# hao-ai-lab/LookaheadDecoding

Measured on NVIDIA H100. Metric: tokens/sec (wall-clock) and accepted-tokens/step, Llama-2-7B W=15 N=5 G=15, higher is better.
Workload: dtype bf16

## Files before the change

lookaheaddecoding_b200/csrc/attn_tc.cu:

```cuda
#include "tc_common.cuh"

#include <cstdlib>
#include <mutex>
#include <type_traits>
#include <unordered_map>

namespace lade {

constexpr int TC_BM = 128;
constexpr int TC_BN = 128;
constexpr int TC_D = 128;
constexpr int TC_STAGES = 3;
constexpr int TC_CONSUMER_THREADS = 256;
constexpr int TC_THREADS = TC_CONSUMER_THREADS + 32;
constexpr int TC_TILE_BYTES = 128 * 128 * 2;
constexpr int TC_HALF_BYTES = TC_TILE_BYTES / 2;
constexpr int TC_SMEM_TILES = TC_TILE_BYTES * (1 + 2 * TC_STAGES);
constexpr int TC_SMEM_BYTES = TC_SMEM_TILES + 256 + 1024;
constexpr float TC_LOG2E = 1.4426950408889634f;
constexpr int TC_MAX_COUNTERS = 16384;

__device__ long long* g_attn_timing = nullptr;
__device__ __forceinline__ long long global_ns() {
  unsigned long long t;
  asm volatile("mov.u64 %0, %%globaltimer;" : "=l"(t));
  return (long long)t;
}
__device__ __forceinline__ int sm_id() {
  int s;
  asm volatile("mov.u32 %0, %%smid;" : "=r"(s));
  return s;
}
#define TC_STAMP(slot, tid) do { if (tbuf && threadIdx.x == (tid)) tbuf[slot] = global_ns(); } while (0)
enum { TS_START = 0, TS_KFULL0 = 1, TS_SFULL0 = 2, TS_OFINAL = 3, TS_STAGED = 4, TS_TICKET = 5, TS_END = 7, TS_SMID = 15 };

template <typename ET> __device__ __forceinline__ float2 unpack2(uint32_t u);
template <> __device__ __forceinline__ float2 unpack2<__nv_bfloat16>(uint32_t u) {
  return make_float2(__uint_as_float(u << 16), __uint_as_float(u & 0xffff0000u));
}
template <> __device__ __forceinline__ float2 unpack2<__half>(uint32_t u) {
  return __half22float2(*reinterpret_cast<__half2*>(&u));
}

template <typename ET>
__device__ __forceinline__ void qk_tile(float (&s)[64], uint32_t sQ_a, uint32_t sK_a, int wg) {
  wg_fence();
#pragma unroll
  for (int kb = 0; kb < 2; ++kb)
#pragma unroll
    for (int k = 0; k < 4; ++k) {
      const uint64_t da = wg_desc(sQ_a + kb * TC_HALF_BYTES + wg * 8192 + k * 32, 16, 1024);
      const uint64_t db = wg_desc(sK_a + kb * TC_HALF_BYTES + k * 32, 16, 1024);
      wgmma_m64n128_ss<ET>(s, da, db, (kb | k) ? 1u : 0u);
    }
  wg_commit();
  wg_wait_all();
  wg_fence_regs(s);
}

template <typename ET>
__device__ __forceinline__ void pv_tile(float (&o)[64], const uint32_t (&p)[32], uint32_t sV_a) {
  wg_fence_regs(o);
  wg_fence();
#pragma unroll
  for (int kk = 0; kk < 8; ++kk) wgmma_m64n128_rs_tb<ET>(o, p + 4 * kk, wg_desc(sV_a + kk * 2048, TC_HALF_BYTES, 1024));
  wg_commit();
  wg_wait_all();
  wg_fence_regs(o);
}

__device__ __forceinline__ void tile_mask(uint32_t (&mb)[2][4], const uint32_t* const (&mrow)[2], const int (&row)[2],
                                          int mask_words, int tile0, int kv_len, int q_len, int is_prefill) {
#pragma unroll
  for (int rr = 0; rr < 2; ++rr)
#pragma unroll
    for (int w = 0; w < 4; ++w)
      mb[rr][w] = (tile0 + 32 * w + 32 <= kv_len)
                      ? 0xffffffffu
                      : visible_bits32(mrow[rr], mask_words, tile0 + 32 * w, kv_len, q_len, is_prefill, row[rr]);
}
__device__ __forceinline__ bool vis(const uint32_t (&mb)[2][4], int rr, int i, int e, int t) {
  return (mb[rr][i >> 2] >> (8 * (i & 3) + 2 * t + e)) & 1u;
}

template <typename ET, bool REF>
__global__ void __launch_bounds__(TC_THREADS, 1)
attn_fwd_tc_kernel(const __grid_constant__ CUtensorMap tmQ, const __grid_constant__ CUtensorMap tmK,
                   const __grid_constant__ CUtensorMap tmV, ET* __restrict__ out,
                   const uint32_t* __restrict__ rowmask, int mask_words, const int* __restrict__ meta, int q_pad,
                   int n_heads, int n_kv_heads, int n_splits, float inv_sqrt_d, int* __restrict__ counters,
                   float2* __restrict__ part_ml, float* __restrict__ part_o) {
  extern __shared__ unsigned char smem_raw[];
  const uint32_t raw_a = smem_u32(smem_raw);
  const uint32_t sQ_a = (raw_a + 1023u) & ~1023u;
  unsigned char* smem = smem_raw + (sQ_a - raw_a);
  const int split = blockIdx.x, h = blockIdx.y, mt = blockIdx.z;
  const int warp = threadIdx.x >> 5, lane = threadIdx.x & 31;

  const int q_len = meta[LADE_M_Q_LEN];
  const int kv_len = meta[LADE_M_KV_LEN];
  const int is_prefill = meta[LADE_M_IS_PREFILL];
  const int T = kv_len + q_len;
  int Tm = T;
  if (is_prefill) Tm = min(T, kv_len + min(q_len, (mt + 1) * TC_BM));
  const int n_tiles = (Tm + TC_BN - 1) / TC_BN;
  const int t_base = n_tiles / n_splits, t_rem = n_tiles - t_base * n_splits;
  const int n_active = n_tiles < n_splits ? n_tiles : n_splits;
  const bool active = split < n_active;
  const int tile_lo = split * t_base + (split < t_rem ? split : t_rem);
  const int my_tiles = active ? t_base + (split < t_rem ? 1 : 0) : 0;
  if (REF && t_base + (t_rem ? 1 : 0) > TC_STAGES) __trap();
  const int hk = h / (n_heads / n_kv_heads);
  const int HD = n_heads * TC_D;
  const long long slab = (long long)n_heads * gridDim.z * TC_BM;
  const long long prow0 = ((long long)h * gridDim.z + mt) * TC_BM;
  const int n_wg = (mt * TC_BM + 64 < q_pad) ? 2 : 1;
  const bool zero_last = active && (tile_lo + my_tiles) * TC_BN > T;
  long long* tbuf = g_attn_timing ? g_attn_timing + 16ll * ((blockIdx.z * gridDim.y + blockIdx.y) * gridDim.x + blockIdx.x) : nullptr;
  TC_STAMP(TS_START, 0);
  if (tbuf && threadIdx.x == 0) tbuf[TS_SMID] = sm_id();
  griddep_launch_dependents();

  uint64_t* bars = reinterpret_cast<uint64_t*>(smem + TC_SMEM_TILES);
  const uint32_t bar0 = smem_u32(bars);
  auto BAR = [&](int i) { return bar0 + 8u * (uint32_t)i; };
  const int B_QFULL = 0, B_KFULL = 1, B_VFULL = 1 + TC_STAGES, B_FREE = 1 + 2 * TC_STAGES, B_VZERO = 1 + 3 * TC_STAGES;
  auto sK_a = [&](int s) { return sQ_a + (uint32_t)TC_TILE_BYTES * (1 + 2 * s); };
  auto sV_a = [&](int s) { return sQ_a + (uint32_t)TC_TILE_BYTES * (2 + 2 * s); };
  auto issue_tile = [&](int j) {
    const int s = j % TC_STAGES;
    const int row0 = (tile_lo + j) * TC_BN;
    mbar_expect_tx(BAR(B_KFULL + s), TC_TILE_BYTES);
    tma_load_3d(sK_a(s), &tmK, BAR(B_KFULL + s), 0, row0, hk);
    tma_load_3d(sK_a(s) + TC_HALF_BYTES, &tmK, BAR(B_KFULL + s), 64, row0, hk);
    mbar_expect_tx(BAR(B_VFULL + s), TC_TILE_BYTES);
    tma_load_3d(sV_a(s), &tmV, BAR(B_VFULL + s), 0, row0, hk);
    tma_load_3d(sV_a(s) + TC_HALF_BYTES, &tmV, BAR(B_VFULL + s), 64, row0, hk);
  };

  if (active && threadIdx.x == TC_CONSUMER_THREADS) {
    mbar_init(BAR(B_QFULL), 1);
    for (int s = 0; s < TC_STAGES; ++s) {
      mbar_init(BAR(B_KFULL + s), 1);
      mbar_init(BAR(B_VFULL + s), 1);
      mbar_init(BAR(B_FREE + s), 4 * n_wg);
    }
    mbar_init(BAR(B_VZERO), 1);
    fence_barrier_init();
    const int n_pre = my_tiles < TC_STAGES ? my_tiles : TC_STAGES;
    int n_old = 0;
    while (n_old < n_pre && (tile_lo + n_old + 1) * TC_BN <= kv_len) ++n_old;
    for (int j = 0; j < n_old; ++j) issue_tile(j);
    griddep_wait();
    mbar_expect_tx(BAR(B_QFULL), TC_TILE_BYTES);
    tma_load_3d(sQ_a, &tmQ, BAR(B_QFULL), 0, mt * TC_BM, h);
    tma_load_3d(sQ_a + TC_HALF_BYTES, &tmQ, BAR(B_QFULL), 64, mt * TC_BM, h);
    for (int j = n_old; j < n_pre; ++j) issue_tile(j);
  }
  __syncthreads();
  griddep_wait();

  const int wg = warp >> 2;
  const int g = lane >> 2, t = lane & 3;
  const int rl[2] = {wg * 64 + (warp & 3) * 16 + g, wg * 64 + (warp & 3) * 16 + g + 8};
  const bool work = active && warp < 8 && wg < n_wg;
  float o[64];
  float m_row[2] = {-INFINITY, -INFINITY}, l_row[2] = {0.f, 0.f};
#pragma unroll
  for (int i = 0; i < 64; ++i) o[i] = 0.f;

  if (warp == 8) {
    if (active) {
      if (lane == 0) {
        for (int j = TC_STAGES; j < my_tiles; ++j) {
          const int s = j % TC_STAGES;
          mbar_wait(BAR(B_FREE + s), ((j / TC_STAGES) - 1) & 1);
          issue_tile(j);
        }
      }
      __syncwarp();
      if (zero_last) {
        const int j = my_tiles - 1, s = j % TC_STAGES;
        const int r0 = T - (tile_lo + j) * TC_BN;
        mbar_wait(BAR(B_VFULL + s), (j / TC_STAGES) & 1);
        unsigned char* pV = smem + TC_TILE_BYTES * (2 + 2 * s);
        const uint4 z = make_uint4(0, 0, 0, 0);
        for (int c = r0 * 8 + lane; c < TC_BN * 8; c += 32) {
          const int r = c >> 3, cc = c & 7;
          *reinterpret_cast<uint4*>(pV + r * 128 + cc * 16) = z;
          *reinterpret_cast<uint4*>(pV + TC_HALF_BYTES + r * 128 + cc * 16) = z;
        }
        fence_proxy_async();
        __syncwarp();
        if (lane == 0) mbar_arrive(BAR(B_VZERO));
      }
    }
    if (REF) {
      cluster_arrive(); cluster_wait();
      cluster_arrive(); cluster_wait();
    }
  } else {
    const int row[2] = {mt * TC_BM + rl[0], mt * TC_BM + rl[1]};
    const uint32_t* const mrow[2] = {
        (row[0] < q_pad && !is_prefill && rowmask != nullptr) ? rowmask + (long long)row[0] * mask_words : nullptr,
        (row[1] < q_pad && !is_prefill && rowmask != nullptr) ? rowmask + (long long)row[1] * mask_words : nullptr};
    auto wait_v = [&](int j) {
      const int s = j % TC_STAGES;
      mbar_wait(BAR(B_VFULL + s), (j / TC_STAGES) & 1);
      if (zero_last && j == my_tiles - 1) mbar_wait(BAR(B_VZERO), 0);
    };
    if (work) mbar_wait(BAR(B_QFULL), 0);
    if (!REF) {
      for (int j = 0; work && j < my_tiles; ++j) {
        const int s = j % TC_STAGES;
        const int tile0 = (tile_lo + j) * TC_BN;
        mbar_wait(BAR(B_KFULL + s), (j / TC_STAGES) & 1);
        if (j == 0) TC_STAMP(TS_KFULL0, 0);
        float sc[64];
        qk_tile<ET>(sc, sQ_a, sK_a(s), wg);
        if (j == 0) TC_STAMP(TS_SFULL0, 0);
        uint32_t mb[2][4];
        tile_mask(mb, mrow, row, mask_words, tile0, kv_len, q_len, is_prefill);
        float off[2];
#pragma unroll
        for (int rr = 0; rr < 2; ++rr) {
          float mx = -INFINITY;
#pragma unroll
          for (int i = 0; i < 16; ++i)
#pragma unroll
            for (int e = 0; e < 2; ++e) mx = fmaxf(mx, vis(mb, rr, i, e, t) ? sc[4 * i + 2 * rr + e] : -INFINITY);
          mx = fmaxf(mx, __shfl_xor_sync(0xffffffffu, mx, 1));
          mx = fmaxf(mx, __shfl_xor_sync(0xffffffffu, mx, 2));
          const float mtile = mx == -INFINITY ? -INFINITY : round_to<ET>(round_to<ET>(mx) * inv_sqrt_d);
          if (mtile > m_row[rr]) {
            const float scale = m_row[rr] == -INFINITY ? 1.f : exp2f((m_row[rr] - mtile) * TC_LOG2E);
            l_row[rr] *= scale;
#pragma unroll
            for (int i = 0; i < 16; ++i) { o[4 * i + 2 * rr] *= scale; o[4 * i + 2 * rr + 1] *= scale; }
            m_row[rr] = mtile;
          }
          off[rr] = m_row[rr] == -INFINITY ? 0.f : m_row[rr] * TC_LOG2E;
        }
        uint32_t pa[32];
#pragma unroll
        for (int i = 0; i < 16; ++i)
#pragma unroll
          for (int rr = 0; rr < 2; ++rr) {
            float r0, r1;
            round_scale_round2<ET>(sc[4 * i + 2 * rr], sc[4 * i + 2 * rr + 1], inv_sqrt_d, r0, r1);
            const float p0 = vis(mb, rr, i, 0, t) ? ex2_approx(r0 * TC_LOG2E - off[rr]) : 0.f;
            const float p1 = vis(mb, rr, i, 1, t) ? ex2_approx(r1 * TC_LOG2E - off[rr]) : 0.f;
            const uint32_t pk = Elem<ET>::pack2(p0, p1);
            const float2 pr = unpack2<ET>(pk);
            l_row[rr] += pr.x + pr.y;
            pa[4 * (i >> 1) + 2 * (i & 1) + rr] = pk;
          }
        wait_v(j);
        pv_tile<ET>(o, pa, sV_a(s));
        __syncwarp();
        if (lane == 0) mbar_arrive(BAR(B_FREE + s));
      }
#pragma unroll
      for (int rr = 0; rr < 2; ++rr) {
        l_row[rr] += __shfl_xor_sync(0xffffffffu, l_row[rr], 1);
        l_row[rr] += __shfl_xor_sync(0xffffffffu, l_row[rr], 2);
      }
    } else {
      float sc[64];
      uint32_t mb[2][4];
      float mx[2] = {-INFINITY, -INFINITY};
      for (int j = 0; work && j < my_tiles; ++j) {
        mbar_wait(BAR(B_KFULL + j), 0);
        qk_tile<ET>(sc, sQ_a, sK_a(j), wg);
        tile_mask(mb, mrow, row, mask_words, (tile_lo + j) * TC_BN, kv_len, q_len, is_prefill);
#pragma unroll
        for (int rr = 0; rr < 2; ++rr)
#pragma unroll
          for (int i = 0; i < 16; ++i)
#pragma unroll
            for (int e = 0; e < 2; ++e) mx[rr] = fmaxf(mx[rr], vis(mb, rr, i, e, t) ? sc[4 * i + 2 * rr + e] : -INFINITY);
      }
      if (work) {
#pragma unroll
        for (int rr = 0; rr < 2; ++rr) {
          mx[rr] = fmaxf(mx[rr], __shfl_xor_sync(0xffffffffu, mx[rr], 1));
          mx[rr] = fmaxf(mx[rr], __shfl_xor_sync(0xffffffffu, mx[rr], 2));
          const float m_split = mx[rr] == -INFINITY ? -INFINITY : round_to<ET>(round_to<ET>(mx[rr]) * inv_sqrt_d);
          if (t == 0) part_ml[split * slab + prow0 + rl[rr]].x = m_split;
        }
      }
      cluster_arrive(); cluster_wait();
      float m_ref[2] = {0.f, 0.f};
      if (work) {
#pragma unroll
        for (int rr = 0; rr < 2; ++rr) {
          float m_all = -INFINITY;
          for (int sp = 0; sp < n_active; ++sp)
            m_all = fmaxf(m_all, ld_global_f2(part_ml + sp * slab + prow0 + rl[rr]).x);
          m_ref[rr] = (m_all == -INFINITY) ? 0.f : m_all;
        }
      }
      auto exps = [&](int j) {
        qk_tile<ET>(sc, sQ_a, sK_a(j), wg);
        tile_mask(mb, mrow, row, mask_words, (tile_lo + j) * TC_BN, kv_len, q_len, is_prefill);
#pragma unroll
        for (int i = 0; i < 16; ++i)
#pragma unroll
          for (int rr = 0; rr < 2; ++rr) {
            float r0, r1;
            round_scale_round2<ET>(sc[4 * i + 2 * rr], sc[4 * i + 2 * rr + 1], inv_sqrt_d, r0, r1);
            sc[4 * i + 2 * rr] = vis(mb, rr, i, 0, t) ? ex2_approx((r0 - m_ref[rr]) * TC_LOG2E) : 0.f;
            sc[4 * i + 2 * rr + 1] = vis(mb, rr, i, 1, t) ? ex2_approx((r1 - m_ref[rr]) * TC_LOG2E) : 0.f;
          }
      };
      float l_part[2] = {0.f, 0.f};
      for (int j = 0; work && j < my_tiles; ++j) {
        exps(j);
#pragma unroll
        for (int rr = 0; rr < 2; ++rr)
#pragma unroll
          for (int i = 0; i < 16; ++i) {
            l_part[rr] += sc[4 * i + 2 * rr];
            l_part[rr] += sc[4 * i + 2 * rr + 1];
          }
      }
      if (work) {
#pragma unroll
        for (int rr = 0; rr < 2; ++rr) {
          l_part[rr] += __shfl_xor_sync(0xffffffffu, l_part[rr], 1);
          l_part[rr] += __shfl_xor_sync(0xffffffffu, l_part[rr], 2);
          if (t == 0) part_ml[split * slab + prow0 + rl[rr]].y = l_part[rr];
        }
      }
      cluster_arrive(); cluster_wait();
      float l_all[2] = {0.f, 0.f};
      if (work) {
#pragma unroll
        for (int rr = 0; rr < 2; ++rr)
          for (int sp = 0; sp < n_active; ++sp) l_all[rr] += ld_global_f2(part_ml + sp * slab + prow0 + rl[rr]).y;
      }
      for (int j = 0; work && j < my_tiles; ++j) {
        exps(j);
        uint32_t pa[32];
#pragma unroll
        for (int i = 0; i < 16; ++i)
#pragma unroll
          for (int rr = 0; rr < 2; ++rr) {
            const float p0 = l_all[rr] > 0.f ? __fdiv_rn(sc[4 * i + 2 * rr], l_all[rr]) : 0.f;
            const float p1 = l_all[rr] > 0.f ? __fdiv_rn(sc[4 * i + 2 * rr + 1], l_all[rr]) : 0.f;
            pa[4 * (i >> 1) + 2 * (i & 1) + rr] = Elem<ET>::pack2(p0, p1);
          }
        wait_v(j);
        pv_tile<ET>(o, pa, sV_a(j));
      }
    }
    TC_STAMP(TS_OFINAL, 0);
    if (work && n_splits == 1) {
#pragma unroll
      for (int rr = 0; rr < 2; ++rr) {
        if (row[rr] >= q_pad) continue;
        const float inv = REF ? 1.f : (l_row[rr] > 0.f ? 1.f / l_row[rr] : 0.f);
        uint32_t* dst = reinterpret_cast<uint32_t*>(out + (long long)row[rr] * HD + h * TC_D + 2 * t);
#pragma unroll
        for (int i = 0; i < 16; ++i) dst[4 * i] = Elem<ET>::pack2(o[4 * i + 2 * rr] * inv, o[4 * i + 2 * rr + 1] * inv);
      }
    }
  }
  if (n_splits == 1) { TC_STAMP(TS_END, 0); return; }
  if (!active) return;

  const int rows_valid = min(TC_BM, q_pad - mt * TC_BM);
  const int per = (rows_valid + n_active - 1) / n_active;
  int* const counter = counters + h * gridDim.z + mt;
  if (n_active > 1) {
    __shared__ int s_last;
    if (work) {
#pragma unroll
      for (int rr = 0; rr < 2; ++rr) {
        if (rl[rr] >= rows_valid) continue;
        float2* po = reinterpret_cast<float2*>(part_o + (split * slab + prow0 + rl[rr]) * TC_D + 2 * t);
#pragma unroll
        for (int i = 0; i < 16; ++i) po[4 * i] = make_float2(o[4 * i + 2 * rr], o[4 * i + 2 * rr + 1]);
        if (!REF && t == 0) part_ml[split * slab + prow0 + rl[rr]] = make_float2(m_row[rr], l_row[rr]);
      }
    }
    TC_STAMP(TS_STAGED, 0);
    __threadfence();
    __syncthreads();
    if (threadIdx.x == 0) s_last = atomicAdd(counter, 1) == n_active - 1;
    __syncthreads();
    TC_STAMP(TS_TICKET, 0);
    if (!s_last) return;
    __threadfence();
    if (threadIdx.x == 0) *counter = 0;
  }
  if (work && n_active == 1) {
#pragma unroll
    for (int rr = 0; rr < 2; ++rr) {
      if (rl[rr] >= rows_valid) continue;
      float wgt = 1.f, inv = 1.f;
      if (!REF) {
        wgt = (m_row[rr] == -INFINITY) ? 0.f : exp2f((m_row[rr] - m_row[rr]) * TC_LOG2E);
        const float lsum = __fmul_rn(l_row[rr], wgt);
        inv = lsum > 0.f ? 1.f / lsum : 0.f;
      }
      uint32_t* dst = reinterpret_cast<uint32_t*>(out + (long long)(mt * TC_BM + rl[rr]) * HD + h * TC_D + 2 * t);
#pragma unroll
      for (int i = 0; i < 16; ++i)
        dst[4 * i] = Elem<ET>::pack2(__fmul_rn(__fmul_rn(o[4 * i + 2 * rr], wgt), inv),
                                     __fmul_rn(__fmul_rn(o[4 * i + 2 * rr + 1], wgt), inv));
    }
  } else if (work) {
    bool valid[2];
    int own[2];
    const float2* pml[2];
    const float2* po[2];
    float mmax[2];
#pragma unroll
    for (int rr = 0; rr < 2; ++rr) {
      valid[rr] = rl[rr] < rows_valid;
      own[rr] = rl[rr] / per;
      pml[rr] = part_ml + prow0 + rl[rr];
      po[rr] = reinterpret_cast<const float2*>(part_o + (prow0 + rl[rr]) * TC_D + 2 * t);
      mmax[rr] = -INFINITY;
      if (!REF && valid[rr]) {
        float mx[8];
#pragma unroll
        for (int s = 0; s < 8; ++s) mx[s] = s < n_active ? __ldcg(pml[rr] + s * slab).x : -INFINITY;
#pragma unroll
        for (int s = 0; s < 8; ++s) mmax[rr] = fmaxf(mmax[rr], mx[s]);
      }
    }
    float acc[2][32], lsum[2] = {0.f, 0.f};
    for (int k = 0; k < n_active; ++k) {
      float2 x[2][16], ml[2];
#pragma unroll
      for (int rr = 0; rr < 2; ++rr) {
        const int s = k == 0 ? own[rr] : (k - 1 < own[rr] ? k - 1 : k);
        if (!valid[rr]) continue;
        if (!REF) ml[rr] = __ldcg(pml[rr] + s * slab);
#pragma unroll
        for (int i = 0; i < 16; ++i) x[rr][i] = __ldcg(po[rr] + s * slab * (TC_D / 2) + 4 * i);
      }
#pragma unroll
      for (int rr = 0; rr < 2; ++rr) {
        if (!valid[rr]) continue;
        if (!REF) {
          const float wgt = (ml[rr].x == -INFINITY) ? 0.f : exp2f((ml[rr].x - mmax[rr]) * TC_LOG2E);
          lsum[rr] = k == 0 ? __fmul_rn(ml[rr].y, wgt) : __fmaf_rn(ml[rr].y, wgt, lsum[rr]);
#pragma unroll
          for (int i = 0; i < 16; ++i) {
            acc[rr][2 * i] = k == 0 ? __fmul_rn(x[rr][i].x, wgt) : __fmaf_rn(x[rr][i].x, wgt, acc[rr][2 * i]);
            acc[rr][2 * i + 1] = k == 0 ? __fmul_rn(x[rr][i].y, wgt) : __fmaf_rn(x[rr][i].y, wgt, acc[rr][2 * i + 1]);
          }
        } else {
#pragma unroll
          for (int i = 0; i < 16; ++i) {
            acc[rr][2 * i] = k == 0 ? x[rr][i].x : __fadd_rn(acc[rr][2 * i], x[rr][i].x);
            acc[rr][2 * i + 1] = k == 0 ? x[rr][i].y : __fadd_rn(acc[rr][2 * i + 1], x[rr][i].y);
          }
        }
      }
    }
#pragma unroll
    for (int rr = 0; rr < 2; ++rr) {
      if (!valid[rr]) continue;
      const float inv = REF ? 1.f : (lsum[rr] > 0.f ? 1.f / lsum[rr] : 0.f);
      uint32_t* dst = reinterpret_cast<uint32_t*>(out + (long long)(mt * TC_BM + rl[rr]) * HD + h * TC_D + 2 * t);
#pragma unroll
      for (int i = 0; i < 16; ++i)
        dst[4 * i] = Elem<ET>::pack2(__fmul_rn(acc[rr][2 * i], inv), __fmul_rn(acc[rr][2 * i + 1], inv));
    }
  }
  TC_STAMP(TS_END, 0);
}

int attn_tc_set_timing_buffer(void* dev_ptr) {
  long long* p = reinterpret_cast<long long*>(dev_ptr);
  cudaError_t e = cudaMemcpyToSymbol(g_attn_timing, &p, sizeof(p));
  if (e != cudaSuccess) { set_cuda_error(e, "cudaMemcpyToSymbol(g_attn_timing)"); return LADE_ECUDA; }
  return LADE_OK;
}

EncodeTiledFn get_encode_fn() {
  static EncodeTiledFn fn = nullptr;
  static bool tried = false;
  if (!tried) {
    tried = true;
    void* p = nullptr;
    cudaDriverEntryPointQueryResult qres;
    if (cudaGetDriverEntryPoint("cuTensorMapEncodeTiled", &p, cudaEnableDefault, &qres) == cudaSuccess &&
        qres == cudaDriverEntryPointSuccess)
      fn = reinterpret_cast<EncodeTiledFn>(p);
  }
  return fn;
}

struct MapKey {
  const void* ptr; int rows; int heads;
  bool operator==(const MapKey& o) const { return ptr == o.ptr && rows == o.rows && heads == o.heads; }
};
struct MapKeyHash {
  size_t operator()(const MapKey& k) const {
    return std::hash<const void*>()(k.ptr) ^ (std::hash<int>()(k.rows) * 31) ^ (std::hash<int>()(k.heads) * 131);
  }
};

static int get_tensor_map(const void* ptr, int rows, int heads, CUtensorMap* out) {
  static std::mutex mu;
  static std::unordered_map<MapKey, CUtensorMap, MapKeyHash> cache;
  std::lock_guard<std::mutex> lock(mu);
  MapKey key{ptr, rows, heads};
  auto it = cache.find(key);
  if (it != cache.end()) { *out = it->second; return LADE_OK; }
  EncodeTiledFn enc = get_encode_fn();
  if (!enc) return LADE_EUNSUPPORTED;
  CUtensorMap tm;
  const cuuint64_t dims[3] = {(cuuint64_t)TC_D, (cuuint64_t)rows, (cuuint64_t)heads};
  const cuuint64_t strides[2] = {(cuuint64_t)TC_D * 2, (cuuint64_t)rows * TC_D * 2};
  const cuuint32_t box[3] = {64, 128, 1};
  const cuuint32_t estr[3] = {1, 1, 1};
  CUresult r = enc(&tm, CU_TENSOR_MAP_DATA_TYPE_BFLOAT16, 3, const_cast<void*>(ptr), dims, strides, box, estr,
                   CU_TENSOR_MAP_INTERLEAVE_NONE, CU_TENSOR_MAP_SWIZZLE_128B, CU_TENSOR_MAP_L2_PROMOTION_L2_256B,
                   CU_TENSOR_MAP_FLOAT_OOB_FILL_NONE);
  if (r != CUDA_SUCCESS) return LADE_ECUDA;
  if (cache.size() > 4096) cache.clear();
  cache.emplace(key, tm);
  *out = tm;
  return LADE_OK;
}

static int g_pdl_override = -1;
int attn_tc_set_pdl(int v) { g_pdl_override = v < 0 ? -1 : (v ? 1 : 0); return LADE_OK; }

static bool pdl_enabled() {
  if (g_pdl_override >= 0) return g_pdl_override != 0;
  static int v = -1;
  if (v < 0) {
    const char* e = getenv("LADE_PDL");
    v = (e && e[0] == '0') ? 0 : 1;
  }
  return v != 0;
}

template <typename ET, bool REF>
static int launch_tc(cudaStream_t stream, const void* q, const void* k_cache, const void* v_cache, void* out,
                     const uint32_t* rowmask, int mask_words, const int32_t* meta, void* scratch, int q_pad, int n_heads,
                     int n_kv_heads, int head_dim, int kv_capacity, int n_splits) {
  const int q_tiles = (q_pad + TC_BM - 1) / TC_BM;
  if ((long long)n_heads * q_tiles > TC_MAX_COUNTERS) return LADE_EUNSUPPORTED;
  if ((reinterpret_cast<uintptr_t>(q) & 15) || (reinterpret_cast<uintptr_t>(k_cache) & 15) ||
      (reinterpret_cast<uintptr_t>(v_cache) & 15))
    return LADE_EINVAL;
  CUtensorMap tmQ, tmK, tmV;
  int rc;
  if ((rc = get_tensor_map(q, q_pad, n_heads, &tmQ)) != LADE_OK) return rc;
  if ((rc = get_tensor_map(k_cache, kv_capacity, n_kv_heads, &tmK)) != LADE_OK) return rc;
  if ((rc = get_tensor_map(v_cache, kv_capacity, n_kv_heads, &tmV)) != LADE_OK) return rc;
  static unsigned long long attr_devs = 0;
  int cur_dev = 0;
  LADE_CUDA_CHECK(cudaGetDevice(&cur_dev));
  if (!((attr_devs >> (cur_dev & 63)) & 1ull)) {
    LADE_CUDA_CHECK(cudaFuncSetAttribute(attn_fwd_tc_kernel<ET, REF>, cudaFuncAttributeMaxDynamicSharedMemorySize, TC_SMEM_BYTES));
    attr_devs |= 1ull << (cur_dev & 63);
  }
  cudaLaunchConfig_t cfg = {};
  cfg.gridDim = dim3(n_splits, n_heads, q_tiles);
  cfg.blockDim = dim3(TC_THREADS);
  cfg.dynamicSmemBytes = TC_SMEM_BYTES;
  cfg.stream = stream;
  cudaLaunchAttribute attr[2];
  int n_attr = 0;
  if (pdl_enabled()) {
    attr[n_attr].id = cudaLaunchAttributeProgrammaticStreamSerialization;
    attr[n_attr++].val.programmaticStreamSerializationAllowed = 1;
  }
  if (REF) {
    attr[n_attr].id = cudaLaunchAttributeClusterDimension;
    attr[n_attr].val.clusterDim.x = n_splits;
    attr[n_attr].val.clusterDim.y = 1;
    attr[n_attr++].val.clusterDim.z = 1;
  }
  cfg.attrs = attr;
  cfg.numAttrs = n_attr;
  const float inv_sqrt_d = 1.0f / sqrtf((float)head_dim);
  int* counters = reinterpret_cast<int*>(scratch);
  float2* part_ml = reinterpret_cast<float2*>(counters + TC_MAX_COUNTERS);
  float* part_o = reinterpret_cast<float*>(part_ml + (size_t)n_splits * n_heads * q_tiles * TC_BM);
  cudaError_t e = cudaLaunchKernelEx(&cfg, attn_fwd_tc_kernel<ET, REF>, tmQ, tmK, tmV, (ET*)out, rowmask, mask_words, meta,
                                     q_pad, n_heads, n_kv_heads, n_splits, inv_sqrt_d, counters, part_ml, part_o);
  if (e != cudaSuccess) { set_cuda_error(e, "cudaLaunchKernelEx(attn_fwd_tc_kernel)"); return LADE_ECUDA; }
  return LADE_OK;
}

template <typename ET>
static int attn_fwd_tc_launch_t(cudaStream_t stream, const void* q, const void* k_cache, const void* v_cache, void* out,
                                const uint32_t* rowmask, int mask_words, const int32_t* meta, void* scratch, int q_pad,
                                int n_heads, int n_kv_heads, int head_dim, int kv_capacity, int kv_bound, int n_splits) {
  (void)kv_bound;
  if (head_dim != TC_D) return LADE_EUNSUPPORTED;
  if (n_splits > 8) n_splits = 8;
  return launch_tc<ET, false>(stream, q, k_cache, v_cache, out, rowmask, mask_words, meta, scratch, q_pad, n_heads,
                              n_kv_heads, head_dim, kv_capacity, n_splits);
}

int attn_fwd_tc_launch(cudaStream_t stream, const void* q, const void* k_cache, const void* v_cache, void* out,
                       const uint32_t* rowmask, int mask_words, const int32_t* meta, void* scratch, int q_pad, int n_heads,
                       int n_kv_heads, int head_dim, int kv_capacity, int kv_bound, int n_splits, int is_f16) {
  if (is_f16)
    return attn_fwd_tc_launch_t<__half>(stream, q, k_cache, v_cache, out, rowmask, mask_words, meta, scratch, q_pad, n_heads,
                                        n_kv_heads, head_dim, kv_capacity, kv_bound, n_splits);
  return attn_fwd_tc_launch_t<__nv_bfloat16>(stream, q, k_cache, v_cache, out, rowmask, mask_words, meta, scratch, q_pad,
                                             n_heads, n_kv_heads, head_dim, kv_capacity, kv_bound, n_splits);
}

template <typename ET>
static int attn_fwd_tc_exact_launch_t(cudaStream_t stream, const void* q, const void* k_cache, const void* v_cache, void* out,
                                      const uint32_t* rowmask, int mask_words, const int32_t* meta, void* scratch, int q_pad,
                                      int n_heads, int n_kv_heads, int head_dim, int kv_capacity, int kv_bound, int n_splits) {
  if (head_dim != TC_D) return LADE_EUNSUPPORTED;
  if (n_splits > 8) n_splits = 8;
  if (kv_bound < 1 || (kv_bound + TC_BN - 1) / TC_BN > TC_STAGES * n_splits) {
    set_error_string("lade_attn_fwd impl 3: kv_bound exceeds 384 * n_splits (every K/V tile of a split must stay in shared memory)");
    return LADE_EUNSUPPORTED;
  }
  return launch_tc<ET, true>(stream, q, k_cache, v_cache, out, rowmask, mask_words, meta, scratch, q_pad, n_heads,
                             n_kv_heads, head_dim, kv_capacity, n_splits);
}

int attn_fwd_tc_exact_launch(cudaStream_t stream, const void* q, const void* k_cache, const void* v_cache, void* out,
                             const uint32_t* rowmask, int mask_words, const int32_t* meta, void* scratch, int q_pad, int n_heads,
                             int n_kv_heads, int head_dim, int kv_capacity, int kv_bound, int n_splits, int is_f16) {
  if (is_f16)
    return attn_fwd_tc_exact_launch_t<__half>(stream, q, k_cache, v_cache, out, rowmask, mask_words, meta, scratch, q_pad,
                                              n_heads, n_kv_heads, head_dim, kv_capacity, kv_bound, n_splits);
  return attn_fwd_tc_exact_launch_t<__nv_bfloat16>(stream, q, k_cache, v_cache, out, rowmask, mask_words, meta, scratch, q_pad,
                                                   n_heads, n_kv_heads, head_dim, kv_capacity, kv_bound, n_splits);
}

}
```

lookaheaddecoding_b200/csrc/tc_common.cuh:

```cuda
#pragma once
#include "common.cuh"

#include <cuda.h>
#include <type_traits>

namespace lade {

__device__ __forceinline__ uint32_t smem_u32(const void* p) { return (uint32_t)__cvta_generic_to_shared(p); }

__device__ __forceinline__ void mbar_init(uint32_t bar, uint32_t count) {
  asm volatile("mbarrier.init.shared::cta.b64 [%0], %1;" ::"r"(bar), "r"(count));
}
__device__ __forceinline__ void mbar_expect_tx(uint32_t bar, uint32_t bytes) {
  asm volatile("mbarrier.arrive.expect_tx.shared::cta.b64 _, [%0], %1;" ::"r"(bar), "r"(bytes) : "memory");
}
__device__ __forceinline__ void mbar_arrive(uint32_t bar) {
  asm volatile("mbarrier.arrive.shared::cta.b64 _, [%0];" ::"r"(bar) : "memory");
}
__device__ __forceinline__ bool mbar_try_wait(uint32_t bar, uint32_t parity) {
  uint32_t ok;
  asm volatile(
      "{\n\t.reg .pred p;\n\t"
      "mbarrier.try_wait.parity.shared::cta.b64 p, [%1], %2;\n\t"
      "selp.u32 %0, 1, 0, p;\n\t}"
      : "=r"(ok) : "r"(bar), "r"(parity) : "memory");
  return ok != 0;
}
__device__ __forceinline__ void mbar_wait(uint32_t bar, uint32_t parity) {
  if (mbar_try_wait(bar, parity)) return;
  const long long t0 = clock64();
  while (!mbar_try_wait(bar, parity)) {
    if (clock64() - t0 > 4000000000LL) __trap();
  }
}
__device__ __forceinline__ void fence_barrier_init() { asm volatile("fence.mbarrier_init.release.cluster;" ::: "memory"); }
__device__ __forceinline__ void fence_proxy_async() { asm volatile("fence.proxy.async.shared::cta;" ::: "memory"); }

__device__ __forceinline__ void tma_load_3d(uint32_t dst, const CUtensorMap* tm, uint32_t bar, int c0, int c1, int c2) {
  asm volatile(
      "cp.async.bulk.tensor.3d.shared::cluster.global.mbarrier::complete_tx::bytes [%0], [%1, {%3, %4, %5}], [%2];"
      ::"r"(dst), "l"(reinterpret_cast<uint64_t>(tm)), "r"(bar), "r"(c0), "r"(c1), "r"(c2) : "memory");
}
__device__ __forceinline__ void tma_prefetch_desc(const CUtensorMap* tm) {
  asm volatile("prefetch.tensormap [%0];" ::"l"(reinterpret_cast<uint64_t>(tm)) : "memory");
}

__device__ __forceinline__ uint64_t wg_desc(uint32_t saddr, uint32_t lbo_bytes, uint32_t sbo_bytes) {
  uint64_t d = 0;
  d |= (uint64_t)((saddr & 0x3FFFF) >> 4);
  d |= (uint64_t)((lbo_bytes >> 4) & 0x3FFF) << 16;
  d |= (uint64_t)((sbo_bytes >> 4) & 0x3FFF) << 32;
  d |= (uint64_t)1 << 62;
  return d;
}
__device__ __forceinline__ void wg_fence() { asm volatile("wgmma.fence.sync.aligned;" ::: "memory"); }
__device__ __forceinline__ void wg_commit() { asm volatile("wgmma.commit_group.sync.aligned;" ::: "memory"); }
__device__ __forceinline__ void wg_wait_all() { asm volatile("wgmma.wait_group.sync.aligned 0;" ::: "memory"); }
template <int N>
__device__ __forceinline__ void wg_fence_regs(float (&d)[N]) {
#pragma unroll
  for (int i = 0; i < N; ++i) asm volatile("" : "+f"(d[i])::"memory");
}

#define LADE_WG_O4(d, i) "+f"(d[i]), "+f"(d[i + 1]), "+f"(d[i + 2]), "+f"(d[i + 3])
#define LADE_WG_O16(d, i) LADE_WG_O4(d, i), LADE_WG_O4(d, i + 4), LADE_WG_O4(d, i + 8), LADE_WG_O4(d, i + 12)
#define LADE_WG_O64(d) LADE_WG_O16(d, 0), LADE_WG_O16(d, 16), LADE_WG_O16(d, 32), LADE_WG_O16(d, 48)
#define LADE_WG_R64 \
  "{%0, %1, %2, %3, %4, %5, %6, %7, %8, %9, %10, %11, %12, %13, %14, %15, %16, %17, %18, %19, %20, %21, %22, %23, " \
  "%24, %25, %26, %27, %28, %29, %30, %31, %32, %33, %34, %35, %36, %37, %38, %39, %40, %41, %42, %43, %44, %45, " \
  "%46, %47, %48, %49, %50, %51, %52, %53, %54, %55, %56, %57, %58, %59, %60, %61, %62, %63}"

template <typename ET>
__device__ __forceinline__ void wgmma_m64n128_ss(float (&d)[64], uint64_t da, uint64_t db, uint32_t accumulate) {
  if constexpr (std::is_same<ET, __half>::value) {
    asm volatile("{\n\t.reg .pred p;\n\tsetp.ne.b32 p, %66, 0;\n\t"
                 "wgmma.mma_async.sync.aligned.m64n128k16.f32.f16.f16 " LADE_WG_R64 ", %64, %65, p, 1, 1, 0, 0;\n\t}"
                 : LADE_WG_O64(d) : "l"(da), "l"(db), "r"(accumulate));
  } else {
    asm volatile("{\n\t.reg .pred p;\n\tsetp.ne.b32 p, %66, 0;\n\t"
                 "wgmma.mma_async.sync.aligned.m64n128k16.f32.bf16.bf16 " LADE_WG_R64 ", %64, %65, p, 1, 1, 0, 0;\n\t}"
                 : LADE_WG_O64(d) : "l"(da), "l"(db), "r"(accumulate));
  }
}
template <typename ET>
__device__ __forceinline__ void wgmma_m64n128_rs_tb(float (&d)[64], const uint32_t* a, uint64_t db) {
  if constexpr (std::is_same<ET, __half>::value) {
    asm volatile("wgmma.mma_async.sync.aligned.m64n128k16.f32.f16.f16 " LADE_WG_R64 ", {%64, %65, %66, %67}, %68, 1, 1, 1, 1;"
                 : LADE_WG_O64(d) : "r"(a[0]), "r"(a[1]), "r"(a[2]), "r"(a[3]), "l"(db));
  } else {
    asm volatile("wgmma.mma_async.sync.aligned.m64n128k16.f32.bf16.bf16 " LADE_WG_R64 ", {%64, %65, %66, %67}, %68, 1, 1, 1, 1;"
                 : LADE_WG_O64(d) : "r"(a[0]), "r"(a[1]), "r"(a[2]), "r"(a[3]), "l"(db));
  }
}
__device__ __forceinline__ void wgmma_m64n32_ss_bf16(float (&d)[16], uint64_t da, uint64_t db) {
  asm volatile("wgmma.mma_async.sync.aligned.m64n32k16.f32.bf16.bf16 "
               "{%0, %1, %2, %3, %4, %5, %6, %7, %8, %9, %10, %11, %12, %13, %14, %15}, %16, %17, 1, 1, 1, 0, 0;"
               : LADE_WG_O16(d, 0) : "l"(da), "l"(db));
}

__device__ __forceinline__ float ex2_approx(float x) {
  float y;
  asm("ex2.approx.ftz.f32 %0, %1;" : "=f"(y) : "f"(x));
  return y;
}
__device__ __forceinline__ void named_bar_sync(int id, int n_threads) {
  asm volatile("bar.sync %0, %1;" ::"r"(id), "r"(n_threads) : "memory");
}
template <typename ET>
__device__ __forceinline__ void round_scale_round2(float a, float b, float c, float& r0, float& r1);
template <>
__device__ __forceinline__ void round_scale_round2<__nv_bfloat16>(float a, float b, float c, float& r0, float& r1) {
  __nv_bfloat162 v1 = __floats2bfloat162_rn(a, b);
  const uint32_t u1 = *reinterpret_cast<uint32_t*>(&v1);
  __nv_bfloat162 v2 = __floats2bfloat162_rn(__uint_as_float(u1 << 16) * c, __uint_as_float(u1 & 0xffff0000u) * c);
  const uint32_t u2 = *reinterpret_cast<uint32_t*>(&v2);
  r0 = __uint_as_float(u2 << 16);
  r1 = __uint_as_float(u2 & 0xffff0000u);
}
template <>
__device__ __forceinline__ void round_scale_round2<__half>(float a, float b, float c, float& r0, float& r1) {
  const float2 f1 = __half22float2(__floats2half2_rn(a, b));
  const float2 f2 = __half22float2(__floats2half2_rn(f1.x * c, f1.y * c));
  r0 = f2.x;
  r1 = f2.y;
}

__device__ __forceinline__ unsigned pack2_bf16(float lo, float hi) {
  __nv_bfloat162 v = __floats2bfloat162_rn(lo, hi);
  return *reinterpret_cast<unsigned*>(&v);
}

__device__ __forceinline__ void griddep_wait() { asm volatile("griddepcontrol.wait;" ::: "memory"); }
__device__ __forceinline__ void griddep_launch_dependents() { asm volatile("griddepcontrol.launch_dependents;" ::: "memory"); }

__device__ __forceinline__ void cluster_arrive() { asm volatile("barrier.cluster.arrive.release.aligned;" ::: "memory"); }
__device__ __forceinline__ void cluster_wait() { asm volatile("barrier.cluster.wait.acquire.aligned;" ::: "memory"); }
__device__ __forceinline__ uint32_t dsmem_addr(uint32_t local_smem_addr, uint32_t cta_rank) {
  uint32_t r;
  asm volatile("mapa.shared::cluster.u32 %0, %1, %2;" : "=r"(r) : "r"(local_smem_addr), "r"(cta_rank));
  return r;
}
__device__ __forceinline__ float4 ld_dsmem_f4(uint32_t addr) {
  float4 v;
  asm volatile("ld.shared::cluster.v4.f32 {%0, %1, %2, %3}, [%4];" : "=f"(v.x), "=f"(v.y), "=f"(v.z), "=f"(v.w) : "r"(addr));
  return v;
}
__device__ __forceinline__ float4 ld_global_f4(const float* p) {
  float4 v;
  asm volatile("ld.global.cg.v4.f32 {%0, %1, %2, %3}, [%4];" : "=f"(v.x), "=f"(v.y), "=f"(v.z), "=f"(v.w) : "l"(p));
  return v;
}
__device__ __forceinline__ float2 ld_global_f2(const float2* p) {
  float2 v;
  asm volatile("ld.global.cg.v2.f32 {%0, %1}, [%2];" : "=f"(v.x), "=f"(v.y) : "l"(p));
  return v;
}


typedef CUresult (*EncodeTiledFn)(CUtensorMap*, CUtensorMapDataType, cuuint32_t, void*, const cuuint64_t*, const cuuint64_t*,
                                  const cuuint32_t*, const cuuint32_t*, CUtensorMapInterleave, CUtensorMapSwizzle,
                                  CUtensorMapL2promotion, CUtensorMapFloatOOBfill);
EncodeTiledFn get_encode_fn();

}
```

Before: 141.1.

## Drop producer warp, issue TMA from consumer, bulk-prefetch split partials for merge

Removes the dedicated producer warp: thread 0 of the consumer group now issues the later K/V TMA loads after freeing each stage, and consumers zero the tail V rows themselves behind a named barrier. Split-KV partial outputs are stored in fragment-native float4 layout, and the last CTA bulk-copies the other splits' partials (O and m/l) into the freed K/V shared memory via cp.async.bulk before merging. The goal is fewer threads and registers per CTA plus a cheaper, smem-served merge. The risk is that putting the producer wait inside the consumer loop serializes loads behind compute, and the slot-overflow path falls back to global loads.

```diff
diff --git a/lookaheaddecoding_b200/csrc/attn_tc.cu b/lookaheaddecoding_b200/csrc/attn_tc.cu
--- a/lookaheaddecoding_b200/csrc/attn_tc.cu
+++ b/lookaheaddecoding_b200/csrc/attn_tc.cu
@@ -11,14 +11,14 @@
 constexpr int TC_BN = 128;
 constexpr int TC_D = 128;
 constexpr int TC_STAGES = 3;
-constexpr int TC_CONSUMER_THREADS = 256;
-constexpr int TC_THREADS = TC_CONSUMER_THREADS + 32;
+constexpr int TC_THREADS = 256;
 constexpr int TC_TILE_BYTES = 128 * 128 * 2;
 constexpr int TC_HALF_BYTES = TC_TILE_BYTES / 2;
 constexpr int TC_SMEM_TILES = TC_TILE_BYTES * (1 + 2 * TC_STAGES);
 constexpr int TC_SMEM_BYTES = TC_SMEM_TILES + 256 + 1024;
 constexpr float TC_LOG2E = 1.4426950408889634f;
 constexpr int TC_MAX_COUNTERS = 16384;
+constexpr int TC_MERGE_SLOTS = 2 * TC_STAGES * TC_TILE_BYTES / (TC_BM * TC_D * 4);
 
 __device__ long long* g_attn_timing = nullptr;
 __device__ __forceinline__ long long global_ns() {
@@ -32,7 +32,8 @@
   return s;
 }
 #define TC_STAMP(slot, tid) do { if (tbuf && threadIdx.x == (tid)) tbuf[slot] = global_ns(); } while (0)
-enum { TS_START = 0, TS_KFULL0 = 1, TS_SFULL0 = 2, TS_OFINAL = 3, TS_STAGED = 4, TS_TICKET = 5, TS_END = 7, TS_SMID = 15 };
+enum { TS_START = 0, TS_KFULL0 = 1, TS_SFULL0 = 2, TS_OFINAL = 3, TS_STAGED = 4, TS_TICKET = 5, TS_FETCHED = 6, TS_END = 7,
+       TS_SMID = 15 };
 
 template <typename ET> __device__ __forceinline__ float2 unpack2(uint32_t u);
 template <> __device__ __forceinline__ float2 unpack2<__nv_bfloat16>(uint32_t u) {
@@ -124,38 +125,44 @@
   uint64_t* bars = reinterpret_cast<uint64_t*>(smem + TC_SMEM_TILES);
   const uint32_t bar0 = smem_u32(bars);
   auto BAR = [&](int i) { return bar0 + 8u * (uint32_t)i; };
-  const int B_QFULL = 0, B_KFULL = 1, B_VFULL = 1 + TC_STAGES, B_FREE = 1 + 2 * TC_STAGES, B_VZERO = 1 + 3 * TC_STAGES;
+  const int B_QFULL = 0, B_KFULL = 1, B_VFULL = 1 + TC_STAGES, B_FREE = 1 + 2 * TC_STAGES, B_MERGE = 1 + 3 * TC_STAGES;
   auto sK_a = [&](int s) { return sQ_a + (uint32_t)TC_TILE_BYTES * (1 + 2 * s); };
   auto sV_a = [&](int s) { return sQ_a + (uint32_t)TC_TILE_BYTES * (2 + 2 * s); };
-  auto issue_tile = [&](int j) {
+  auto issue_k = [&](int j) {
     const int s = j % TC_STAGES;
     const int row0 = (tile_lo + j) * TC_BN;
     mbar_expect_tx(BAR(B_KFULL + s), TC_TILE_BYTES);
     tma_load_3d(sK_a(s), &tmK, BAR(B_KFULL + s), 0, row0, hk);
     tma_load_3d(sK_a(s) + TC_HALF_BYTES, &tmK, BAR(B_KFULL + s), 64, row0, hk);
+  };
+  auto issue_v = [&](int j) {
+    const int s = j % TC_STAGES;
+    const int row0 = (tile_lo + j) * TC_BN;
     mbar_expect_tx(BAR(B_VFULL + s), TC_TILE_BYTES);
     tma_load_3d(sV_a(s), &tmV, BAR(B_VFULL + s), 0, row0, hk);
     tma_load_3d(sV_a(s) + TC_HALF_BYTES, &tmV, BAR(B_VFULL + s), 64, row0, hk);
   };
-
-  if (active && threadIdx.x == TC_CONSUMER_THREADS) {
+  auto issue_tile = [&](int j) { issue_k(j); issue_v(j); };
+
+  if (active && threadIdx.x == 0) {
     mbar_init(BAR(B_QFULL), 1);
     for (int s = 0; s < TC_STAGES; ++s) {
       mbar_init(BAR(B_KFULL + s), 1);
       mbar_init(BAR(B_VFULL + s), 1);
       mbar_init(BAR(B_FREE + s), 4 * n_wg);
     }
-    mbar_init(BAR(B_VZERO), 1);
+    mbar_init(BAR(B_MERGE), 1);
     fence_barrier_init();
     const int n_pre = my_tiles < TC_STAGES ? my_tiles : TC_STAGES;
-    int n_old = 0;
-    while (n_old < n_pre && (tile_lo + n_old + 1) * TC_BN <= kv_len) ++n_old;
-    for (int j = 0; j < n_old; ++j) issue_tile(j);
+    const bool k0_old = (tile_lo + 1) * TC_BN <= kv_len;
+    if (k0_old) issue_k(0);
     griddep_wait();
     mbar_expect_tx(BAR(B_QFULL), TC_TILE_BYTES);
     tma_load_3d(sQ_a, &tmQ, BAR(B_QFULL), 0, mt * TC_BM, h);
     tma_load_3d(sQ_a + TC_HALF_BYTES, &tmQ, BAR(B_QFULL), 64, mt * TC_BM, h);
-    for (int j = n_old; j < n_pre; ++j) issue_tile(j);
+    if (!k0_old) issue_k(0);
+    issue_v(0);
+    for (int j = 1; j < n_pre; ++j) issue_tile(j);
   }
   __syncthreads();
   griddep_wait();
@@ -163,43 +170,13 @@
   const int wg = warp >> 2;
   const int g = lane >> 2, t = lane & 3;
   const int rl[2] = {wg * 64 + (warp & 3) * 16 + g, wg * 64 + (warp & 3) * 16 + g + 8};
-  const bool work = active && warp < 8 && wg < n_wg;
+  const bool work = active && wg < n_wg;
   float o[64];
   float m_row[2] = {-INFINITY, -INFINITY}, l_row[2] = {0.f, 0.f};
 #pragma unroll
   for (int i = 0; i < 64; ++i) o[i] = 0.f;
 
-  if (warp == 8) {
-    if (active) {
-      if (lane == 0) {
-        for (int j = TC_STAGES; j < my_tiles; ++j) {
-          const int s = j % TC_STAGES;
-          mbar_wait(BAR(B_FREE + s), ((j / TC_STAGES) - 1) & 1);
-          issue_tile(j);
-        }
-      }
-      __syncwarp();
-      if (zero_last) {
-        const int j = my_tiles - 1, s = j % TC_STAGES;
-        const int r0 = T - (tile_lo + j) * TC_BN;
-        mbar_wait(BAR(B_VFULL + s), (j / TC_STAGES) & 1);
-        unsigned char* pV = smem + TC_TILE_BYTES * (2 + 2 * s);
-        const uint4 z = make_uint4(0, 0, 0, 0);
-        for (int c = r0 * 8 + lane; c < TC_BN * 8; c += 32) {
-          const int r = c >> 3, cc = c & 7;
-          *reinterpret_cast<uint4*>(pV + r * 128 + cc * 16) = z;
-          *reinterpret_cast<uint4*>(pV + TC_HALF_BYTES + r * 128 + cc * 16) = z;
-        }
-        fence_proxy_async();
-        __syncwarp();
-        if (lane == 0) mbar_arrive(BAR(B_VZERO));
-      }
-    }
-    if (REF) {
-      cluster_arrive(); cluster_wait();
-      cluster_arrive(); cluster_wait();
-    }
-  } else {
+  {
     const int row[2] = {mt * TC_BM + rl[0], mt * TC_BM + rl[1]};
     const uint32_t* const mrow[2] = {
         (row[0] < q_pad && !is_prefill && rowmask != nullptr) ? rowmask + (long long)row[0] * mask_words : nullptr,
@@ -207,7 +184,18 @@
     auto wait_v = [&](int j) {
       const int s = j % TC_STAGES;
       mbar_wait(BAR(B_VFULL + s), (j / TC_STAGES) & 1);
-      if (zero_last && j == my_tiles - 1) mbar_wait(BAR(B_VZERO), 0);
+      if (zero_last && j == my_tiles - 1) {
+        const int r0 = T - (tile_lo + j) * TC_BN;
+        unsigned char* pV = smem + TC_TILE_BYTES * (2 + 2 * s);
+        const uint4 z = make_uint4(0, 0, 0, 0);
+        for (int c = r0 * 8 + (int)threadIdx.x; c < TC_BN * 8; c += 128 * n_wg) {
+          const int r = c >> 3, cc = c & 7;
+          *reinterpret_cast<uint4*>(pV + r * 128 + cc * 16) = z;
+          *reinterpret_cast<uint4*>(pV + TC_HALF_BYTES + r * 128 + cc * 16) = z;
+        }
+        fence_proxy_async();
+        named_bar_sync(1, 128 * n_wg);
+      }
     };
     if (work) mbar_wait(BAR(B_QFULL), 0);
     if (!REF) {
@@ -257,8 +245,14 @@
           }
         wait_v(j);
         pv_tile<ET>(o, pa, sV_a(s));
-        __syncwarp();
-        if (lane == 0) mbar_arrive(BAR(B_FREE + s));
+        if (j + TC_STAGES < my_tiles) {
+          __syncwarp();
+          if (lane == 0) mbar_arrive(BAR(B_FREE + s));
+          if (threadIdx.x == 0) {
+            mbar_wait(BAR(B_FREE + s), (j / TC_STAGES) & 1);
+            issue_tile(j + TC_STAGES);
+          }
+        }
       }
 #pragma unroll
       for (int rr = 0; rr < 2; ++rr) {
@@ -372,22 +366,41 @@
   const int rows_valid = min(TC_BM, q_pad - mt * TC_BM);
   const int per = (rows_valid + n_active - 1) / n_active;
   int* const counter = counters + h * gridDim.z + mt;
+  auto part_frag = [&](int s) {
+    return reinterpret_cast<float4*>(part_o + (s * slab + prow0) * TC_D) + warp * 16 * 32 + lane;
+  };
   if (n_active > 1) {
     __shared__ int s_last;
     if (work) {
-#pragma unroll
-      for (int rr = 0; rr < 2; ++rr) {
-        if (rl[rr] >= rows_valid) continue;
-        float2* po = reinterpret_cast<float2*>(part_o + (split * slab + prow0 + rl[rr]) * TC_D + 2 * t);
-#pragma unroll
-        for (int i = 0; i < 16; ++i) po[4 * i] = make_float2(o[4 * i + 2 * rr], o[4 * i + 2 * rr + 1]);
-        if (!REF && t == 0) part_ml[split * slab + prow0 + rl[rr]] = make_float2(m_row[rr], l_row[rr]);
-      }
+      float4* po = part_frag(split);
+#pragma unroll
+      for (int i = 0; i < 16; ++i) po[32 * i] = make_float4(o[4 * i], o[4 * i + 1], o[4 * i + 2], o[4 * i + 3]);
+#pragma unroll
+      for (int rr = 0; rr < 2; ++rr)
+        if (!REF && t == 0 && rl[rr] < rows_valid) part_ml[split * slab + prow0 + rl[rr]] = make_float2(m_row[rr], l_row[rr]);
     }
     TC_STAMP(TS_STAGED, 0);
     __threadfence();
     __syncthreads();
-    if (threadIdx.x == 0) s_last = atomicAdd(counter, 1) == n_active - 1;
+    if (threadIdx.x == 0) {
+      const bool last = atomicAdd(counter, 1) == n_active - 1;
+      if (last) {
+        __threadfence();
+        fence_proxy_async_global();
+        const int n_slots = min(n_active - 1, TC_MERGE_SLOTS);
+        const uint32_t o_bytes = (uint32_t)n_wg * 64 * TC_D * 4;
+        mbar_expect_tx(BAR(B_MERGE), n_slots * o_bytes + (REF ? 0u : (uint32_t)(n_active - 1) * TC_BM * 8));
+        for (int s = 0, slot = 0; s < n_active; ++s) {
+          if (s == split) continue;
+          if (slot < TC_MERGE_SLOTS)
+            bulk_load(sQ_a + TC_TILE_BYTES + slot * (TC_BM * TC_D * 4), part_o + (s * slab + prow0) * TC_D, o_bytes,
+                      BAR(B_MERGE));
+          if (!REF) bulk_load(sQ_a + slot * (TC_BM * 8), part_ml + s * slab + prow0, TC_BM * 8, BAR(B_MERGE));
+          ++slot;
+        }
+      }
+      s_last = last;
+    }
     __syncthreads();
     TC_STAMP(TS_TICKET, 0);
     if (!s_last) return;
@@ -411,65 +424,83 @@
                                      __fmul_rn(__fmul_rn(o[4 * i + 2 * rr + 1], wgt), inv));
     }
   } else if (work) {
-    bool valid[2];
-    int own[2];
-    const float2* pml[2];
-    const float2* po[2];
-    float mmax[2];
-#pragma unroll
-    for (int rr = 0; rr < 2; ++rr) {
-      valid[rr] = rl[rr] < rows_valid;
-      own[rr] = rl[rr] / per;
-      pml[rr] = part_ml + prow0 + rl[rr];
-      po[rr] = reinterpret_cast<const float2*>(part_o + (prow0 + rl[rr]) * TC_D + 2 * t);
-      mmax[rr] = -INFINITY;
-      if (!REF && valid[rr]) {
-        float mx[8];
-#pragma unroll
-        for (int s = 0; s < 8; ++s) mx[s] = s < n_active ? __ldcg(pml[rr] + s * slab).x : -INFINITY;
-#pragma unroll
-        for (int s = 0; s < 8; ++s) mmax[rr] = fmaxf(mmax[rr], mx[s]);
-      }
-    }
-    float acc[2][32], lsum[2] = {0.f, 0.f};
-    for (int k = 0; k < n_active; ++k) {
-      float2 x[2][16], ml[2];
+    mbar_wait(BAR(B_MERGE), 0);
+    TC_STAMP(TS_FETCHED, 0);
+    const float4* so = reinterpret_cast<const float4*>(smem + TC_TILE_BYTES) + warp * 16 * 32 + lane;
+    const float2* sml = reinterpret_cast<const float2*>(smem);
+    auto slot_of = [&](int s) { return s - (s > split ? 1 : 0); };
+    auto fetch = [&](int s, float4 (&x)[16], bool both) {
+      float4 v[16];
+      if (s == split) {
+#pragma unroll
+        for (int i = 0; i < 16; ++i) v[i] = make_float4(o[4 * i], o[4 * i + 1], o[4 * i + 2], o[4 * i + 3]);
+      } else if (slot_of(s) < TC_MERGE_SLOTS) {
+#pragma unroll
+        for (int i = 0; i < 16; ++i) v[i] = so[slot_of(s) * (TC_BM * TC_D / 4) + 32 * i];
+      } else {
+        const float4* p = part_frag(s);
+#pragma unroll
+        for (int i = 0; i < 16; ++i) v[i] = __ldcg(p + 32 * i);
+      }
+#pragma unroll
+      for (int i = 0; i < 16; ++i) {
+        if (both) x[i] = v[i];
+        else { x[i].z = v[i].z; x[i].w = v[i].w; }
+      }
+    };
+    auto fetch_ml = [&](int s, int rr) {
+      return s == split ? make_float2(m_row[rr], l_row[rr]) : sml[slot_of(s) * TC_BM + rl[rr]];
+    };
+    const bool valid1 = rl[1] < rows_valid;
+    if (rl[0] < rows_valid) {
+      const int own[2] = {rl[0] / per, valid1 ? rl[1] / per : rl[0] / per};
+      float mmax[2] = {-INFINITY, -INFINITY};
+      if (!REF)
+        for (int s = 0; s < n_active; ++s) {
+          mmax[0] = fmaxf(mmax[0], fetch_ml(s, 0).x);
+          mmax[1] = fmaxf(mmax[1], fetch_ml(s, 1).x);
+        }
+      float acc[2][32], lsum[2] = {0.f, 0.f};
+      for (int k = 0; k < n_active; ++k) {
+        int sk[2];
+#pragma unroll
+        for (int rr = 0; rr < 2; ++rr)
+          sk[rr] = k == 0 ? own[rr] : (k - 1 < own[rr] ? k - 1 : k);
+        float4 x[16];
+        fetch(sk[0], x, true);
+        if (sk[1] != sk[0]) fetch(sk[1], x, false);
+#pragma unroll
+        for (int rr = 0; rr < 2; ++rr) {
+          if (rr == 1 && !valid1) continue;
+          if (!REF) {
+            const float2 ml = fetch_ml(sk[rr], rr);
+            const float wgt = (ml.x == -INFINITY) ? 0.f : exp2f((ml.x - mmax[rr]) * TC_LOG2E);
+            lsum[rr] = k == 0 ? __fmul_rn(ml.y, wgt) : __fmaf_rn(ml.y, wgt, lsum[rr]);
+#pragma unroll
+            for (int i = 0; i < 16; ++i) {
+              const float x0 = rr ? x[i].z : x[i].x, x1 = rr ? x[i].w : x[i].y;
+              acc[rr][2 * i] = k == 0 ? __fmul_rn(x0, wgt) : __fmaf_rn(x0, wgt, acc[rr][2 * i]);
+              acc[rr][2 * i + 1] = k == 0 ? __fmul_rn(x1, wgt) : __fmaf_rn(x1, wgt, acc[rr][2 * i + 1]);
+            }
+          } else {
+#pragma unroll
+            for (int i = 0; i < 16; ++i) {
+              const float x0 = rr ? x[i].z : x[i].x, x1 = rr ? x[i].w : x[i].y;
+              acc[rr][2 * i] = k == 0 ? x0 : __fadd_rn(acc[rr][2 * i], x0);
+              acc[rr][2 * i + 1] = k == 0 ? x1 : __fadd_rn(acc[rr][2 * i + 1], x1);
+            }
+          }
+        }
+      }
 #pragma unroll
       for (int rr = 0; rr < 2; ++rr) {
-        const int s = k == 0 ? own[rr] : (k - 1 < own[rr] ? k - 1 : k);
-        if (!valid[rr]) continue;
-        if (!REF) ml[rr] = __ldcg(pml[rr] + s * slab);
-#pragma unroll
-        for (int i = 0; i < 16; ++i) x[rr][i] = __ldcg(po[rr] + s * slab * (TC_D / 2) + 4 * i);
-      }
-#pragma unroll
-      for (int rr = 0; rr < 2; ++rr) {
-        if (!valid[rr]) continue;
-        if (!REF) {
-          const float wgt = (ml[rr].x == -INFINITY) ? 0.f : exp2f((ml[rr].x - mmax[rr]) * TC_LOG2E);
-          lsum[rr] = k == 0 ? __fmul_rn(ml[rr].y, wgt) : __fmaf_rn(ml[rr].y, wgt, lsum[rr]);
-#pragma unroll
-          for (int i = 0; i < 16; ++i) {
-            acc[rr][2 * i] = k == 0 ? __fmul_rn(x[rr][i].x, wgt) : __fmaf_rn(x[rr][i].x, wgt, acc[rr][2 * i]);
-            acc[rr][2 * i + 1] = k == 0 ? __fmul_rn(x[rr][i].y, wgt) : __fmaf_rn(x[rr][i].y, wgt, acc[rr][2 * i + 1]);
-          }
-        } else {
-#pragma unroll
-          for (int i = 0; i < 16; ++i) {
-            acc[rr][2 * i] = k == 0 ? x[rr][i].x : __fadd_rn(acc[rr][2 * i], x[rr][i].x);
-            acc[rr][2 * i + 1] = k == 0 ? x[rr][i].y : __fadd_rn(acc[rr][2 * i + 1], x[rr][i].y);
-          }
-        }
-      }
-    }
-#pragma unroll
-    for (int rr = 0; rr < 2; ++rr) {
-      if (!valid[rr]) continue;
-      const float inv = REF ? 1.f : (lsum[rr] > 0.f ? 1.f / lsum[rr] : 0.f);
-      uint32_t* dst = reinterpret_cast<uint32_t*>(out + (long long)(mt * TC_BM + rl[rr]) * HD + h * TC_D + 2 * t);
-#pragma unroll
-      for (int i = 0; i < 16; ++i)
-        dst[4 * i] = Elem<ET>::pack2(__fmul_rn(acc[rr][2 * i], inv), __fmul_rn(acc[rr][2 * i + 1], inv));
+        if (rr == 1 && !valid1) continue;
+        const float inv = REF ? 1.f : (lsum[rr] > 0.f ? 1.f / lsum[rr] : 0.f);
+        uint32_t* dst = reinterpret_cast<uint32_t*>(out + (long long)(mt * TC_BM + rl[rr]) * HD + h * TC_D + 2 * t);
+#pragma unroll
+        for (int i = 0; i < 16; ++i)
+          dst[4 * i] = Elem<ET>::pack2(__fmul_rn(acc[rr][2 * i], inv), __fmul_rn(acc[rr][2 * i + 1], inv));
+      }
     }
   }
   TC_STAMP(TS_END, 0);
diff --git a/lookaheaddecoding_b200/csrc/tc_common.cuh b/lookaheaddecoding_b200/csrc/tc_common.cuh
--- a/lookaheaddecoding_b200/csrc/tc_common.cuh
+++ b/lookaheaddecoding_b200/csrc/tc_common.cuh
@@ -35,6 +35,12 @@
 }
 __device__ __forceinline__ void fence_barrier_init() { asm volatile("fence.mbarrier_init.release.cluster;" ::: "memory"); }
 __device__ __forceinline__ void fence_proxy_async() { asm volatile("fence.proxy.async.shared::cta;" ::: "memory"); }
+__device__ __forceinline__ void fence_proxy_async_global() { asm volatile("fence.proxy.async.global;" ::: "memory"); }
+
+__device__ __forceinline__ void bulk_load(uint32_t dst, const void* src, uint32_t bytes, uint32_t bar) {
+  asm volatile("cp.async.bulk.shared::cluster.global.mbarrier::complete_tx::bytes [%0], [%1], %2, [%3];"
+               ::"r"(dst), "l"(reinterpret_cast<uint64_t>(src)), "r"(bytes), "r"(bar) : "memory");
+}
 
 __device__ __forceinline__ void tma_load_3d(uint32_t dst, const CUtensorMap* tm, uint32_t bar, int c0, int c1, int c2) {
   asm volatile(
```

New measurement: 145.6 (median of 6 runs). +3.1%, better.
